# google-research/frame-interpolation

Measured on NVIDIA H100. Metric: interpolated_frames_per_sec_1080p, higher is better.
Workload: dtype f16x2-split (activations/weights as fp16 hi+lo planes; fp32 accumulate)

## Files before the change

### frame_interpolation_b200/csrc/film_conv.h

```cpp
#pragma once
#include <cuda.h>
#include <stdint.h>

#include "film_common.cuh"

namespace film {

constexpr int kMaxSrc = 4;
constexpr int kMaxTaps = 9;
constexpr int kChunk = 64;
constexpr int kTileM = 128;

struct ConvSrc {
  const sp_t* hi;
  const sp_t* lo;
  int C;
  int c_off;
  int nchunk;
  int bswap;
};

struct alignas(64) ConvProblem {
  CUtensorMap tm_a_hi[kMaxSrc];
  CUtensorMap tm_a_lo[kMaxSrc];
  CUtensorMap tm_w_hi;
  CUtensorMap tm_w_lo;
  CUtensorMap tm_w_hi_half;
  CUtensorMap tm_w_lo_half;
  ConvSrc src[kMaxSrc];
  int nsrc;
  int B, H, W;
  int tile_h, tile_w;
  int tiles_y, tiles_x;
  int ntaps;
  int tap_dy[kMaxTaps], tap_dx[kMaxTaps];
  int kchunk;
  int ktot;
// ... 2 lines not shown
  const float* bias;
  int cout;
  int act;
  sp_t* out_hi;
  sp_t* out_lo;
  int out_C, out_c_off;
  int out_H, out_W;
  int out_sy, out_sx, out_oy, out_ox;
  int epi_mode;
  const float* head_w3;
  const float* head_b3;
  int crop_y, crop_x, crop_h, crop_w;
  int64_t crop_pitch;
  const float* head_w4;
  const float* head_b4;
  const float* head_vup;
  float* head_res;
  float* head_v;
  int v2_resident;
  int v2_na, v2_nw;
  int v2_grid;
  int v2_part_lo, v2_part_hi;
  sp_t* pool_hi;
  sp_t* pool_lo;
  int pool_C;
  int group;
  int pair;
  int halo;
  int bn;
  int passes;
  int straight;
  int out_lo_skip;
  int pxn;
};

cudaError_t launch_conv_tc(const ConvProblem* d_prob, const ConvProblem& h_prob, cudaStream_t st);
cudaError_t launch_conv_simt(const ConvProblem* d_prob, const ConvProblem& h_prob, cudaStream_t st);
cudaError_t conv_tc_configure();
bool conv3x3_tc_plan(ConvProblem& h_prob, int num_sms);
void conv3x3_tc_pick_tile(int H, int W, int B, int cout, int kc, int passes, int ktot, int epi_mode, int num_sms,
                          int& tile_h, int& tile_w);
cudaError_t launch_conv3x3_tc(const ConvProblem* d_prob, const ConvProblem& h_prob, cudaStream_t st);
cudaError_t conv3x3_tc_configure();
}
```

### frame_interpolation_b200/csrc/film_conv3x3_tc.cu

```cuda
#include <cuda.h>
#include <cuda_runtime.h>
#include <stdint.h>

#include <type_traits>

#include "film_conv.h"
#include "film_tc_ptx.cuh"

namespace film {
namespace {
using namespace tc;

constexpr int kConsumers = 256;
constexpr int kThreads = kConsumers + 128;
__host__ __device__ constexpr int a_plane_bytes(int kc, int th, int tw) { return (th + 2) * tw * kc * 2; }
__host__ __device__ constexpr int a_stage_bytes(int kc, int th, int tw) { return 2 * a_plane_bytes(kc, th, tw); }
constexpr int kHaloW = 10;
__host__ __device__ constexpr int halo_box_bytes(int kc, int th) { return (th + 2) * kHaloW * kc * 2; }
__host__ __device__ constexpr int halo_plane_bytes(int kc, int th) { return (halo_box_bytes(kc, th) + 1023) & ~1023; }
__host__ __device__ constexpr int a_stage_bytes_h(int kc, int th, int tw, int halo, int planes = 2) {
  return planes * (halo ? halo_plane_bytes(kc, th) : a_plane_bytes(kc, th, tw));
}
constexpr int kMaxRing = 8;
constexpr int kSmemLimit = 227 * 1024;
// ... 537 lines not shown
              f0 = leaky(f0);
              f1 = leaky(f1);
            }
            if (valid[h]) {
              sp_t* oh = out_hi + opix[h] * out_C + out_c_off + n0;
              if (lo_skip) {
                *reinterpret_cast<uint32_t*>(oh + c) = pack2_hi(f0, f1);
              } else {
                sp_t* ol = out_lo + opix[h] * out_C + out_c_off + n0;
                uint32_t hi, lo;
                split_pack2(f0, f1, hi, lo);
                *reinterpret_cast<uint32_t*>(oh + c) = hi;
                *reinterpret_cast<uint32_t*>(ol + c) = lo;
              }
            }
            if (do_pool) {
              a[h][0] = f0 + __shfl_xor_sync(0xffffffffu, f0, 4);
              a[h][1] = f1 + __shfl_xor_sync(0xffffffffu, f1, 4);
            }
          }
          if (do_pool && pool_ok) {
            uint32_t hi, lo;
            split_pack2((a[0][0] + a[1][0]) * 0.25f, (a[0][1] + a[1][1]) * 0.25f, hi, lo);
            *reinterpret_cast<uint32_t*>(pool_hi + ppix * pool_C + n0 + c) = hi;
            *reinterpret_cast<uint32_t*>(pool_lo + ppix * pool_C + n0 + c) = lo;
          }
        }
      }
    }
  }
  leave();
}

int smem_bytes_for(const ConvProblem& h, int bn) {
  const int nkb = h.ktot / h.kchunk;
  const int planes = h.passes == 1 ? 1 : 2;
  const int w = h.v2_resident ? nkb * w_tap_bytes(bn, h.kchunk, planes) : h.v2_nw * w_tap_bytes(bn, h.kchunk, planes);
  return h.v2_na * a_stage_bytes_h(h.kchunk, h.tile_h, h.tile_w, h.halo, planes) + w + kFixedBytes +
         epi_scratch_bytes(h.epi_mode, h.pxn);
}

}

int conv_tc_block_n(int cout);

namespace {
bool ring_depths(int kc, int tile_h, int tile_w, int halo, int planes, int bn, int cout, int ktot, int epi_mode, int pxn,
                 int& resident, int& na, int& nw) {
  const int wtap = w_tap_bytes(bn, kc, planes);
  const int w_all = (ktot / kc) * wtap;
  const int kLimit = kSmemLimit - epi_scratch_bytes(epi_mode, pxn);
  const int kAStage = a_stage_bytes_h(kc, tile_h, tile_w, halo, planes);
  if (cout <= bn && w_all + 2 * kAStage + kFixedBytes <= kLimit) {
    resident = 1;
    const int n = (kLimit - kFixedBytes - w_all) / kAStage;
    const int n_max = halo ? 3 : 6;
    na = n > n_max ? n_max : n;
    nw = 1;
    return true;
  }
  resident = 0;
  na = halo ? 2 : (bn >= 128 ? 2 : 3);
  int n = (kLimit - kFixedBytes - na * kAStage) / wtap;
  if (n < 2 && na > 2) {
    na = 2;
    n = (kLimit - kFixedBytes - na * kAStage) / wtap;
// ... 75 lines not shown
    if (h.v2_na < 2 || (!h.v2_resident && h.v2_nw < 2)) return cudaErrorInvalidValue;
    if (kPxN && (h.pair || h.tile_h != 32 || h.tile_w != 8 || h.epi_mode != 0)) return cudaErrorInvalidValue;
    const bool partial = h.v2_part_hi > h.v2_part_lo;
    const int idx = (partial ? 8 : 0) | (h.halo ? 4 : 0) | (h.passes == 1 ? 2 : 0) | (h.v2_resident && h.straight ? 1 : 0);
    if (!h.pair) {
      kFn[idx]<<<h.v2_grid, kThreads, smem_bytes_for(h, BN), st>>>(d_prob);
      return cudaGetLastError();
    }
    cudaLaunchConfig_t cfg = {};
    cudaLaunchAttribute attr[1];
    attr[0].id = cudaLaunchAttributeClusterDimension;
    attr[0].val.clusterDim.x = 2;
    attr[0].val.clusterDim.y = 1;
    attr[0].val.clusterDim.z = 1;
    cfg.gridDim = dim3(h.v2_grid);
    cfg.blockDim = dim3(kThreads);
    cfg.dynamicSmemBytes = smem_bytes_for(h, BN);
    cfg.stream = st;
    cfg.attrs = attr;
    cfg.numAttrs = 1;
    return cudaLaunchKernelEx(&cfg, kFn[idx], d_prob);
  }
};

cudaError_t conv3x3_tc_configure() {
  cudaError_t e;
#define FILM_CFG(BN, KC)                        \
  e = Variants<BN, KC>::configure();            \
  if (e != cudaSuccess) return e;
  FILM_CFG(32, 64) FILM_CFG(64, 64) FILM_CFG(128, 64) FILM_CFG(256, 64) FILM_CFG(32, 32) FILM_CFG(64, 32)
#undef FILM_CFG
  e = Variants<64, 64, true>::configure();
  if (e != cudaSuccess) return e;
  return cudaSuccess;
}

cudaError_t launch_conv3x3_tc(const ConvProblem* d_prob, const ConvProblem& h, cudaStream_t st) {
  const int bn = h.bn;
  if (h.kchunk == 32) {
    if (bn == 32) return Variants<32, 32>::launch(d_prob, h, st);
    if (bn == 64) return Variants<64, 32>::launch(d_prob, h, st);
    return cudaErrorInvalidValue;
  }
  switch (bn) {
    case 256: return Variants<256, 64>::launch(d_prob, h, st);
    case 128: return Variants<128, 64>::launch(d_prob, h, st);
    case 64: return h.pxn ? Variants<64, 64, true>::launch(d_prob, h, st) : Variants<64, 64>::launch(d_prob, h, st);
    default: return Variants<32, 64>::launch(d_prob, h, st);
  }
}

}
```

### frame_interpolation_b200/csrc/film_engine.cu

```cuda
#include <cuda.h>
#include <cuda_runtime.h>

#include <algorithm>
#include <cmath>
#include <cstdio>
#include <cstdlib>
#include <cstring>
#include <functional>
#include <map>
#include <memory>
#include <string>
#include <vector>

#include "../../include/film_b200.h"
#include "film_conv.h"
#include "film_kernels.h"
#include "film_pack.h"

namespace film {
int conv_tc_block_n(int cout);

constexpr int kLevels = 7, kFusionLevels = 5, kSpecialized = 3, kSubLevels = 4, kFilters = 64;
static const int kFlowFilters[4] = {32, 64, 128, 256};
static const char* kPredictorNames[4] = {"flow_predictor_0", "flow_predictor_1", "flow_predictor_2",
// ... 22 lines not shown
static std::string stage_name(int s) {
  static const char* fe[] = {"fe_i0_k01", "fe_i0_k23", "fe_i0_k45", "fe_i0_k67", "fe_i1", "fe_i2", "fe_i3p"};
  if (s < 0 || s >= ST_COUNT) return "";
  if (s < ST_FLOW_L0) return fe[s];
  if (s < ST_FUS) return "flow_L" + std::to_string(s - ST_FLOW_L0);
  return "fus" + std::to_string((s - ST_FUS) / 3) + "_c" + std::to_string((s - ST_FUS) % 3);
}
static int fe_stage(int image_level, int conv_k) {
  if (image_level == 0) return ST_FE_I0_K01 + conv_k / 2;
  return image_level == 1 ? ST_FE_I1 : image_level == 2 ? ST_FE_I2 : ST_FE_I3P;
}
constexpr uint32_t kDefaultOnepassMask =
    (1u << ST_FE_I0_K23) | (1u << ST_FE_I0_K45) | (1u << ST_FE_I0_K67) |
    (0x1Fu << ST_FLOW_L0) | (0x3Fu << (ST_FUS + 6));

struct Options {
  int conv_impl = 0;
  int use_graph = 1;
  int keep_debug = 0;
  int time_ops = 0;
  int use_lanes = 0;
  int conv3x3_v2 = 1;
  int conv3x3_2cta = 0;
  int conv3x3_halo = 3;
  int conv3x3_pxn = 1;
  int onepass_mask = (int)kDefaultOnepassMask;
  int fe_conv0_tc = 0;
  int fuse_rgb_head = 1;
  int fuse_flow_head = 1;
  int plane_skip = 1;
  int mma_straight = 1;
  int arena_reuse = 1;
  int any_size = 0;
};

static int as_given(int v) { return v; }
static int as_bool(int v) { return v ? 1 : 0; }
static int clamp_0_2(int v) { return v < 0 ? 0 : (v > 2 ? 2 : v); }
static int stage_bits(int v) { return (int)((uint32_t)v & ((1u << ST_COUNT) - 1u)); }
struct OptionRow {
  const char* name;
  int Options::*field;
  int (*normalise)(int);
  const char* env;
  bool plan_key;
};
static const OptionRow kOptions[] = {
    {"conv_impl", &Options::conv_impl, as_given, nullptr, true},
    {"use_graph", &Options::use_graph, as_given, nullptr, false},
    {"keep_debug", &Options::keep_debug, as_given, nullptr, true},
    {"time_ops", &Options::time_ops, as_given, nullptr, false},
    {"use_lanes", &Options::use_lanes, as_given, nullptr, true},
    {"conv3x3_v2", &Options::conv3x3_v2, as_given, nullptr, true},
    {"conv3x3_2cta", &Options::conv3x3_2cta, as_given, "FILM_2CTA", true},
    {"conv3x3_halo", &Options::conv3x3_halo, as_given, "FILM_HALO", true},
    {"conv3x3_pxn", &Options::conv3x3_pxn, clamp_0_2, nullptr, true},
    {"onepass_mask", &Options::onepass_mask, stage_bits, "FILM_ONEPASS", true},
    {"fe_conv0_tc", &Options::fe_conv0_tc, as_bool, "FILM_FE0_TC", true},
    {"fuse_rgb_head", &Options::fuse_rgb_head, as_bool, "FILM_RGB_FUSE", true},
    {"fuse_flow_head", &Options::fuse_flow_head, clamp_0_2, "FILM_FLOW_HEAD_FUSE", true},
    {"plane_skip", &Options::plane_skip, as_bool, "FILM_PLANE_SKIP", true},
    {"mma_straight", &Options::mma_straight, as_bool, "FILM_STRAIGHT", true},
    {"arena_reuse", &Options::arena_reuse, as_bool, "FILM_ARENA_REUSE", true},
    {"any_size", &Options::any_size, as_bool, nullptr, false},
};
static const OptionRow& option_row(const char* name) {
  for (const OptionRow& r : kOptions)
    if (!strcmp(r.name, name)) return r;
  throw Error{FILM_ERR_ARG, std::string("unknown option ") + name};
}

#define FILM_CUDA(expr)                                                                       \
  do {                                                                                        \
    cudaError_t e__ = (expr);                                                                 \
    if (e__ != cudaSuccess)                                                                   \
      throw Error{FILM_ERR_CUDA, std::string(#expr) + ": " + cudaGetErrorString(e__)};        \
  } while (0)

struct HostTensor {
  std::vector<int> dims;
  std::vector<float> data;
};
typedef std::map<std::string, HostTensor> WeightMap;

static WeightMap read_weight_file(const char* path) {
  FILE* f = fopen(path, "rb");
  if (!f) throw Error{FILM_ERR_WEIGHTS, std::string("cannot open weight file ") + path};
  WeightMap m;
  auto fail = [&](const char* why) {
    fclose(f);
    throw Error{FILM_ERR_WEIGHTS, std::string(path) + ": " + why};
  };
  char magic[8];
  if (fread(magic, 1, 8, f) != 8 || memcmp(magic, "FILMW1\0\0", 8) != 0) fail("bad magic");
  uint32_t n;
  if (fread(&n, 4, 1, f) != 1) fail("truncated");
  for (uint32_t i = 0; i < n; ++i) {
// ... 50 lines not shown
}
static float sp_to_f32(uint16_t h) {
#ifdef FILM_SPLIT_FP16
  __half v;
  memcpy(&v, &h, 2);
  return __half2float(v);
#else
  return bf16_to_f32(h);
#endif
}

struct PackedConv {
  sp_t* w_hi = nullptr;
  sp_t* w_lo = nullptr;
  float* bias = nullptr;
  int cout = 0, ktot = 0, cin_ref = 0;
  int kchunk = kChunk;
  std::vector<int> src_chunks;
  std::vector<int> src_ksteps;
  sp_t* pxn_hi = nullptr;
  sp_t* pxn_lo = nullptr;
  int pxn_ktot = 0;
  int ntaps = 0;
  int tap_dy[kMaxTaps], tap_dx[kMaxTaps];
};

struct TapSpec {
  int dy, dx;
  std::vector<std::pair<int, int>> terms;
};

static PackedConv pack_conv(const HostTensor& kernel, const HostTensor& bias,
                            const std::vector<std::vector<int>>& src_maps,
                            const std::vector<TapSpec>& taps, std::vector<void*>& allocs, int chunk = kChunk) {
  const int kw = kernel.dims[1], cin = kernel.dims[2], cout = kernel.dims[3];
  PackedConv pc;
  pc.cout = cout;
  pc.cin_ref = cin;
  pc.kchunk = chunk;
  pc.ntaps = (int)taps.size();
  for (size_t t = 0; t < taps.size(); ++t) {
    pc.tap_dy[t] = taps[t].dy;
    pc.tap_dx[t] = taps[t].dx;
  }
  int ktot = 0;
  for (auto& sm : src_maps) {
    if (sm.size() % chunk) throw Error{FILM_ERR_WEIGHTS, "source channel map not a multiple of the K chunk"};
    pc.src_chunks.push_back((int)sm.size() / chunk);
    int ks = 1;
    for (size_t i = 0; i < sm.size(); ++i)
      if (sm[i] >= 0) ks = std::max(ks, (int)(i % chunk) / 16 + 1);
    pc.src_ksteps.push_back(ks);
    ktot += (int)sm.size() * (int)taps.size();
  }
  pc.ktot = ktot;
  std::vector<uint16_t> hi((size_t)cout * ktot), lo((size_t)cout * ktot);
  int kbase = 0;
  for (auto& sm : src_maps) {
    const int nchunk = (int)sm.size() / chunk;
    for (int ch = 0; ch < nchunk; ++ch) {
      for (size_t t = 0; t < taps.size(); ++t, kbase += chunk) {
        for (int c = 0; c < chunk; ++c) {
          const int ref = sm[ch * chunk + c];
          for (int n = 0; n < cout; ++n) {
            float w = 0.f;
            if (ref >= 0) {
              if (ref >= cin) throw Error{FILM_ERR_WEIGHTS, "channel map out of range"};
              for (auto& term : taps[t].terms)
                w += kernel.data[(((size_t)term.first * kw + term.second) * cin + ref) * cout + n];
            }
            const uint16_t h = f32_to_sp(w);
            const uint16_t l = f32_to_sp(w - sp_to_f32(h));
            hi[(size_t)n * ktot + kbase + c] = h;
            lo[(size_t)n * ktot + kbase + c] = l;
          }
        }
      }
    }
  }
  auto upload = [&](const std::vector<uint16_t>& v) {
    sp_t* d;
    FILM_CUDA(cudaMalloc(&d, v.size() * 2));
    allocs.push_back(d);
    FILM_CUDA(cudaMemcpy(d, v.data(), v.size() * 2, cudaMemcpyHostToDevice));
    return d;
  };
  pc.w_hi = upload(hi);
  pc.w_lo = upload(lo);
  pc.pxn_hi = pc.w_hi;
  pc.pxn_lo = pc.w_lo;
  pc.pxn_ktot = ktot;
  std::vector<int> packed;
  for (int ks : pc.src_ksteps) packed.push_back(taps.size() == 9 && chunk == kChunk && ks == 1);
  if (std::count(packed.begin(), packed.end(), 1)) {
    pc.pxn_hi = upload(pack_dx_blocks(hi, cout, ktot, chunk, pc.src_chunks, packed, pc.pxn_ktot));
    pc.pxn_lo = upload(pack_dx_blocks(lo, cout, ktot, chunk, pc.src_chunks, packed, pc.pxn_ktot));
  }
  FILM_CUDA(cudaMalloc(&pc.bias, cout * 4));
  allocs.push_back(pc.bias);
  FILM_CUDA(cudaMemcpy(pc.bias, bias.data.data(), cout * 4, cudaMemcpyHostToDevice));
  return pc;
}

static std::vector<TapSpec> taps_3x3() {
  std::vector<TapSpec> t;
  for (int kx = 0; kx < 3; ++kx)
    for (int ky = 0; ky < 3; ++ky) t.push_back({ky - 1, kx - 1, {{ky, kx}}});
  return t;
}
static std::vector<TapSpec> taps_up2x2(int py, int px) {
  std::vector<TapSpec> t;
  for (int dy = 0; dy <= py; ++dy)
    for (int dx = 0; dx <= px; ++dx) {
      TapSpec s{dy, dx, {}};
      for (int fy = 0; fy < 2; ++fy)
        for (int fx = 0; fx < 2; ++fx)
          if ((py + fy) / 2 == dy && (px + fx) / 2 == dx) s.terms.push_back({fy, fx});
      t.push_back(s);
    }
  return t;
}
static std::vector<int> iota_map(int start, int n, int padded) {
  std::vector<int> m(padded, -1);
  for (int i = 0; i < n; ++i) m[i] = start + i;
  return m;
}
static std::vector<int> side_map(int C) {
  std::vector<int> m(kChunk, -1);
  for (int c = 0; c < 3; ++c) m[c] = c;
  for (int c = 0; c < 3; ++c) m[3 + c] = 3 + C + c;
  m[6] = 6 + 2 * C;
  m[7] = 7 + 2 * C;
  m[8] = 8 + 2 * C;
  m[9] = 9 + 2 * C;
  return m;
}

struct Model {
  std::vector<void*> allocs;
  float *conv0_w = nullptr, *conv0_b = nullptr;
  PackedConv fe[8];
  PackedConv fe0_3x3;
  PackedConv flow[4][3];
  PackedConv flow_c3[4];
  float *flow_w3[4], *flow_b3[4], *flow_w4[4], *flow_b4[4];
  PackedConv fus_up[4][4];
  PackedConv fus_up_2x2[4];
  PackedConv fus_c1[4], fus_c2[4];
  float *rgb_w = nullptr, *rgb_b = nullptr;

  float* upload(const HostTensor& t) {
    float* d;
    FILM_CUDA(cudaMalloc(&d, t.data.size() * 4));
    allocs.push_back(d);
    FILM_CUDA(cudaMemcpy(d, t.data.data(), t.data.size() * 4, cudaMemcpyHostToDevice));
    return d;
  }

  void load(const WeightMap& w) {
    const std::string fe_pre = "feat_net/sub_extractor/cfeat_conv_";
    conv0_w = upload(get_tensor(w, fe_pre + "0/kernel", {3, 3, 3, 64}));
    conv0_b = upload(get_tensor(w, fe_pre + "0/bias", {64}));
    {
      HostTensor k0 = get_tensor(w, fe_pre + "0/kernel", {3, 3, 3, 64});
      k0.dims = {1, 1, 27, 64};
      fe[0] = pack_conv(k0, get_tensor(w, fe_pre + "0/bias", {64}), {iota_map(0, 27, 32)},
                        {TapSpec{0, 0, {{0, 0}}}}, allocs, 32);
      fe0_3x3 = pack_conv(get_tensor(w, fe_pre + "0/kernel", {3, 3, 3, 64}), get_tensor(w, fe_pre + "0/bias", {64}),
                          {iota_map(0, 3, 32)}, taps_3x3(), allocs, 32);
    }
    int cin = 64;
    for (int k = 1; k < 8; ++k) {
      const int c = kFilters << (k / 2);
      fe[k] = pack_conv(get_tensor(w, fe_pre + std::to_string(k) + "/kernel", {3, 3, cin, c}),
                        get_tensor(w, fe_pre + std::to_string(k) + "/bias", {c}),
                        {iota_map(0, cin, cin)}, taps_3x3(), allocs);
      cin = c;
    }
    for (int p = 0; p < 4; ++p) {
      const std::string pre = std::string("predict_flow/") + kPredictorNames[p] + "/conv_";
      const int nf = kFlowFilters[p], C = feat_channels(p);
      flow[p][0] = pack_conv(get_tensor(w, pre + "0/kernel", {3, 3, 2 * C, nf}),
                             get_tensor(w, pre + "0/bias", {nf}),
                             {iota_map(0, C, C), iota_map(C, C, C)}, taps_3x3(), allocs);
      const int kc = nf < kChunk ? 32 : kChunk;
      for (int k = 1; k < 3; ++k)
        flow[p][k] = pack_conv(get_tensor(w, pre + std::to_string(k) + "/kernel", {3, 3, nf, nf}),
                               get_tensor(w, pre + std::to_string(k) + "/bias", {nf}),
                               {iota_map(0, nf, round_up(nf, kc))}, taps_3x3(), allocs, kc);
      flow_c3[p] = pack_conv(get_tensor(w, pre + "3/kernel", {1, 1, nf, nf / 2}),
                             get_tensor(w, pre + "3/bias", {nf / 2}), {iota_map(0, nf, round_up(nf, kc))},
                             {TapSpec{0, 0, {{0, 0}}}}, allocs, kc);
      flow_w3[p] = upload(get_tensor(w, pre + "3/kernel", {1, 1, nf, nf / 2}));
      flow_b3[p] = upload(get_tensor(w, pre + "3/bias", {nf / 2}));
      flow_w4[p] = upload(get_tensor(w, pre + "4/kernel", {1, 1, nf / 2, 2}));
      flow_b4[p] = upload(get_tensor(w, pre + "4/bias", {2}));
    }
    for (int i = 0; i < kFusionLevels - 1; ++i) {
      const std::string pre = "fusion/level_" + std::to_string(i) + "/conv_";
      const int nf = fusion_filters(i), C = feat_channels(i);
      const bool from_pyr = (i == kFusionLevels - 2);
      const int Cc = feat_channels(i + 1);
      const int coarse_c = from_pyr ? 2 * (3 + Cc) + 4 : fusion_filters(i + 1);
      const HostTensor& k0 = get_tensor(w, pre + "0/kernel", {2, 2, coarse_c, nf});
      const HostTensor& b0 = get_tensor(w, pre + "0/bias", {nf});
      std::vector<std::vector<int>> up_src;
      if (from_pyr)
        up_src = {iota_map(3, Cc, Cc), iota_map(6 + Cc, Cc, Cc), side_map(Cc)};
      else
        up_src = {iota_map(0, coarse_c, coarse_c)};
      for (int py = 0; py < 2; ++py)
        for (int px = 0; px < 2; ++px)
          fus_up[i][py * 2 + px] = pack_conv(k0, b0, up_src, taps_up2x2(py, px), allocs);
      fus_up_2x2[i] = pack_conv(k0, b0, up_src, {{0, 0, {{0, 0}}}, {0, 1, {{0, 1}}}, {1, 0, {{1, 0}}}, {1, 1, {{1, 1}}}},
                                allocs);
      const int a_c = 2 * (3 + C) + 4;
      fus_c1[i] = pack_conv(get_tensor(w, pre + "1/kernel", {3, 3, a_c + nf, nf}),
                            get_tensor(w, pre + "1/bias", {nf}),
                            {iota_map(3, C, C), iota_map(6 + C, C, C), side_map(C),
                             iota_map(a_c, nf, round_up(nf, kChunk))},
                            taps_3x3(), allocs);
      fus_c2[i] = pack_conv(get_tensor(w, pre + "2/kernel", {3, 3, nf, nf}),
                            get_tensor(w, pre + "2/bias", {nf}),
                            {iota_map(0, nf, round_up(nf, kChunk))}, taps_3x3(), allocs);
    }
    rgb_w = upload(get_tensor(w, "fusion/output_conv/kernel", {1, 1, 64, 3}));
    rgb_b = upload(get_tensor(w, "fusion/output_conv/bias", {3}));
  }
  ~Model() {
    for (void* p : allocs) cudaFree(p);
  }
};

typedef CUresult (*EncodeTiledFn)(CUtensorMap*, CUtensorMapDataType, cuuint32_t, void*, const cuuint64_t*,
                                  const cuuint64_t*, const cuuint32_t*, const cuuint32_t*,
                                  CUtensorMapInterleave, CUtensorMapSwizzle, CUtensorMapL2promotion,
                                  CUtensorMapFloatOOBfill);
static EncodeTiledFn get_encode_fn() {
  static EncodeTiledFn fn = nullptr;
  if (!fn) {
    void* p = nullptr;
    cudaDriverEntryPointQueryResult qres;
    FILM_CUDA(cudaGetDriverEntryPoint("cuTensorMapEncodeTiled", &p, cudaEnableDefault, &qres));
    if (qres != cudaDriverEntryPointSuccess || !p)
      throw Error{FILM_ERR_CUDA, "cuTensorMapEncodeTiled entry point not available"};
    fn = (EncodeTiledFn)p;
// ... 290 lines not shown
                                              tag + ")"};
      cp.v2_part_lo = ab;
      cp.v2_part_hi = ab + pc.src_chunks[s] * nst;
    }
  }
  const size_t idx = P.h_probs.size();
  P.h_probs.push_back(cp);
  double k_issued = 0;
  for (size_t si = 0; si < pc.src_chunks.size(); ++si)
    k_issued += (double)pc.src_chunks[si] * pc.ntaps * (v2 ? pc.src_ksteps[si] * 16 : pc.kchunk);
  P.mma_flops += (double)cp.passes * 2.0 * (double)cp.B * cp.tiles_y * cp.tiles_x * (cp.tile_h * cp.tile_w) * k_issued *
                 (double)(((pc.cout + bn - 1) / bn) * bn);
  double alg_bytes = 0;
  {
    const double px = (double)cp.B * cp.H * cp.W, planes_in = cp.passes == 1 ? 1.0 : 2.0;
    for (size_t si = 0; si < pc.src_chunks.size(); ++si) alg_bytes += px * pc.src_chunks[si] * pc.kchunk * 2.0 * planes_in;
    if (out) alg_bytes += px * pc.cout * 2.0 * (cp.out_lo_skip ? 1.0 : 2.0);
    if (pool_out) alg_bytes += px / 4.0 * pc.cout * 4.0;
    if (epi_mode == 2) alg_bytes += px * 12.0;
    if (!out && epi_mode != 2) alg_bytes += px * 24.0;
    alg_bytes += (double)pc.cout * ktot * 2.0 * planes_in;
  }
  P.last_conv_bytes = alg_bytes;
  if (no_op) return idx;
  Plan* pp = &P;
  const int impl = o.conv_impl;
  P.add_op(0, tag, [pp, idx, impl, v2](cudaStream_t st) {
    if (impl == 1) return launch_conv_simt(pp->d_probs + idx, pp->h_probs[idx], st);
    return v2 ? launch_conv3x3_tc(pp->d_probs + idx, pp->h_probs[idx], st)
              : launch_conv_tc(pp->d_probs + idx, pp->h_probs[idx], st);
  }, 2.0 * ref_macs_per_px * (double)cp.B * cp.H * cp.W, alg_bytes);
  P.ops.back().form = impl == 1 ? "simt" : !v2 ? "tc" : cp.pxn ? "3x3_pxn" : "3x3";
  return idx;
}

static void padded_size(int h, int w, int align, int& H, int& W, int& off_y, int& off_x) {
  int ph = 0, pw = 0;
  if (align > 0) {
    ph = (h % align) ? align - h % align : 0;
    pw = (w % align) ? align - w % align : 0;
  }
  H = h + ph;
  W = w + pw;
  off_y = ph / 2;
  off_x = pw / 2;
}

static std::unique_ptr<Plan> build_plan(const Model& M, int h, int w, int align, const Options& opt, int num_sms) {
  std::unique_ptr<Plan> pl(new Plan);
  Plan& P = *pl;
  P.opt = opt;
  P.reuse = !opt.keep_debug && !opt.use_lanes && opt.arena_reuse;
  const bool fuse_rgb = opt.conv_impl == 0 && opt.conv3x3_v2 && opt.fuse_rgb_head && !opt.keep_debug;
  P.h = h;
  P.w = w;
  P.num_sms = num_sms;
  padded_size(h, w, align, P.H, P.W, P.off_y, P.off_x);
  int Hs[kLevels], Ws[kLevels];
  for (int l = 0; l < kLevels; ++l) {
    Hs[l] = P.H >> l;
    Ws[l] = P.W >> l;
  }
  if (Hs[kLevels - 2] < 2 || Ws[kLevels - 2] < 2) throw Error{FILM_ERR_ARG, "frame too small"};

  P.xin = P.alloc<float>((int64_t)2 * h * w * 3, true);
  P.xout = P.alloc<float>((int64_t)h * w * 3, true);
// ... 238 lines not shown
    const int nf = fusion_filters(i), hh = Hs[i], ww = Ws[i];
    const int cpad = round_up(nf, kChunk);
    SplitBuf* up = P.split(1, hh, ww, cpad);
    std::vector<SrcRef> up_src;
    if (i == kFusionLevels - 2)
      up_src = {{batch_view(wf[i + 1], 0), 0}, {batch_view(wf[i + 1], 1), 0}, {side[i + 1], 0}};
    else
      up_src = {{net, 0}};
    if (hh != 2 * Hs[i + 1] || ww != 2 * Ws[i + 1]) {
      const bool hi_only = P.hi_only(ST_FUS + 3 * i);
      std::vector<std::pair<const SplitBuf*, SplitBuf*>> jobs;
      if (i == kFusionLevels - 2) {
        jobs.push_back({wf[i + 1], P.split(2, hh, ww, wf[i + 1]->C)});
        jobs.push_back({side[i + 1], P.split(1, hh, ww, side[i + 1]->C)});
        up_src = {{batch_view(jobs[0].second, 0), 0}, {batch_view(jobs[0].second, 1), 0}, {jobs[1].second, 0}};
      } else {
        jobs.push_back({net, P.split(1, hh, ww, net->C)});
        up_src = {{jobs[0].second, 0}};
      }
      double rbytes = 0;
      for (auto& j : jobs) rbytes += (double)j.second->pixels() * j.second->C * (hi_only ? 4.0 : 8.0);
      P.add_op(2, "fusion_resize@L" + std::to_string(i), [jobs, hi_only](cudaStream_t st) {
        for (auto& j : jobs) {
          const SplitBuf *s = j.first, *d = j.second;
          const cudaError_t e = launch_resize_nearest(s->hi, s->lo, s->C, 0, s->B, s->H, s->W, d->hi, d->lo, d->C, 0, d->H,
                                                      d->W, d->C, hi_only, st);
          if (e != cudaSuccess) return e;
        }
        return cudaSuccess;
      }, 0, rbytes);
      add_conv(P, "fusion_up@L" + std::to_string(i), 4.0 * M.fus_up_2x2[i].cin_ref * nf, M.fus_up_2x2[i], up_src, 0, up, 0,
               ST_FUS + 3 * i, ST_FUS + 3 * i + 1);
      for (auto& j : jobs) P.release(j.second);
    } else if (opt.conv_impl == 0) {
      size_t first = 0;
      for (int py = 0; py < 2; ++py)
        for (int px = 0; px < 2; ++px) {
          const size_t ci = add_conv(P, "", 0, M.fus_up[i][py * 2 + px], up_src, 0, up, 0, ST_FUS + 3 * i, ST_FUS + 3 * i + 1, 2, 2,
                                     py, px, nullptr, true);
          if (py == 0 && px == 0) first = ci;
        }
      P.h_probs[first].group = 4;
      const double up_bytes = 4.0 * P.last_conv_bytes;
      Plan* pq = &P;
      const double fl = 2.0 * 16.0 * M.fus_up[i][0].cin_ref * nf * (double)Hs[i + 1] * Ws[i + 1];
      P.add_op(0, "fusion_up@L" + std::to_string(i), [pq, first](cudaStream_t st) {
        return launch_conv_tc(pq->d_probs + first, pq->h_probs[first], st);
      }, fl, up_bytes);
    } else {
      for (int py = 0; py < 2; ++py)
        for (int px = 0; px < 2; ++px)
          add_conv(P, "fusion_up" + std::to_string(py * 2 + px) + "@L" + std::to_string(i),
                   4.0 * M.fus_up[i][0].cin_ref * nf, M.fus_up[i][py * 2 + px], up_src, 0, up, 0, ST_FUS + 3 * i,
                   ST_FUS + 3 * i + 1, 2, 2, py, px);
    }
    SplitBuf* f1 = P.split(1, hh, ww, cpad);
    SplitBuf* f2 = (fuse_rgb && i == 0) ? nullptr : P.split(1, hh, ww, cpad);
    add_conv(P, "fusion_conv1@L" + std::to_string(i), 9.0 * M.fus_c1[i].cin_ref * nf, M.fus_c1[i],
             {{batch_view(wf[i], 0), 0}, {batch_view(wf[i], 1), 0}, {side[i], 0}, {up, 0}}, 1, f1, 0, ST_FUS + 3 * i + 1,
             ST_FUS + 3 * i + 2);
    if (fuse_rgb && i == 0) {
      const size_t ci = add_conv(P, "fusion_conv2+rgb@L0", 9.0 * nf * nf + 64.0 * 3, M.fus_c2[i], {{f1, 0}}, 1, nullptr, 0,
                                 ST_FUS + 3 * i + 2, ST_NONE, 1, 1, 0, 0, nullptr, false, 2);
      ConvProblem& hp = P.h_probs[ci];
      if (hp.cout != 64 || hp.bn != 64) throw Error{FILM_ERR_UNSUPPORTED, "RGB-head epilogue expects a 64-channel N tile"};
      hp.head_w4 = M.rgb_w;
      hp.head_b4 = M.rgb_b;
      hp.head_v = P.xout;
      hp.crop_y = P.off_y;
      hp.crop_x = P.off_x;
      hp.crop_h = P.h;
      hp.crop_w = P.w;
      hp.crop_pitch = (int64_t)P.w * 3;
    } else {
      add_conv(P, "fusion_conv2@L" + std::to_string(i), 9.0 * nf * nf, M.fus_c2[i], {{f1, 0}}, 1, f2, 0, ST_FUS + 3 * i + 2,
               i > 0 ? ST_FUS + 3 * (i - 1) : ST_NONE);
    }
    if (i == kFusionLevels - 2) P.release(wf[i + 1]);
    else P.release(net);
    P.release(wf[i]);
    P.release(up);
// ... 772 lines not shown
```

### frame_interpolation_b200/csrc/film_pack.h

```cpp
#pragma once
#include <stdint.h>

#include <vector>

namespace film {

inline std::vector<uint16_t> pack_dx_blocks(const std::vector<uint16_t>& per_tap, int cout, int ktot, int chunk,
                                            const std::vector<int>& src_chunks, const std::vector<int>& packed,
                                            int& ktot_out) {
  ktot_out = ktot;
  for (size_t s = 0; s < src_chunks.size(); ++s)
    if (packed[s]) ktot_out -= src_chunks[s] * 6 * chunk;
  std::vector<uint16_t> out((size_t)cout * ktot_out, 0);
  for (int n = 0; n < cout; ++n) {
    const uint16_t* src = per_tap.data() + (size_t)n * ktot;
    uint16_t* dst = out.data() + (size_t)n * ktot_out;
    for (size_t s = 0; s < src_chunks.size(); ++s)
      for (int ch = 0; ch < src_chunks[s]; ++ch, src += 9 * chunk) {
        if (!packed[s]) {
          for (int k = 0; k < 9 * chunk; ++k) *dst++ = src[k];
          continue;
        }
        for (int t = 0; t < 9; ++t)
          for (int c = 0; c < 16; ++c) dst[(t / 3) * chunk + (t % 3) * 16 + c] = src[t * chunk + c];
        dst += 3 * chunk;
      }
  }
  return out;
}

}
```

Before: 26.01.

## Add dedicated up2x tensor-core kernel sharing input tiles across all four phases

Adds a warp-specialized TMA+wgmma kernel for the fusion upsample conv that loads one input halo tile per channel chunk and computes all four sub-pixel output classes from it. Weights are repacked so each 256-wide N tile pulls only the taps its classes need. The epilogue writes interleaved 2x outputs with vectorized stores after a quad transpose. This replaces the grouped per-class path and is meant to cut repeated activation loads and launch/tile overhead, at the cost of more shared-memory weight traffic and a new, complex code path enabled by default.

```diff
diff --git a/frame_interpolation_b200/csrc/film_conv.h b/frame_interpolation_b200/csrc/film_conv.h
--- a/frame_interpolation_b200/csrc/film_conv.h
+++ b/frame_interpolation_b200/csrc/film_conv.h
@@ -3,6 +3,7 @@
 #include <stdint.h>
 
 #include "film_common.cuh"
+#include "film_pack.h"
 
 namespace film {
 
@@ -71,6 +72,7 @@
   int straight;
   int out_lo_skip;
   int pxn;
+  Up2xPlan up;
 };
 
 cudaError_t launch_conv_tc(const ConvProblem* d_prob, const ConvProblem& h_prob, cudaStream_t st);
@@ -81,4 +83,6 @@
                           int& tile_h, int& tile_w);
 cudaError_t launch_conv3x3_tc(const ConvProblem* d_prob, const ConvProblem& h_prob, cudaStream_t st);
 cudaError_t conv3x3_tc_configure();
+bool up2x_tc_plan(ConvProblem& h_prob, int num_sms);
+cudaError_t launch_up2x_tc(const ConvProblem* d_prob, const ConvProblem& h_prob, cudaStream_t st);
 }
diff --git a/frame_interpolation_b200/csrc/film_conv3x3_tc.cu b/frame_interpolation_b200/csrc/film_conv3x3_tc.cu
--- a/frame_interpolation_b200/csrc/film_conv3x3_tc.cu
+++ b/frame_interpolation_b200/csrc/film_conv3x3_tc.cu
@@ -593,6 +593,271 @@
   leave();
 }
 
+constexpr int kUpBoxW = 9, kUpBoxH = 17;
+constexpr int kUpAPlane = (kUpBoxW * kUpBoxH * 128 + 1023) & ~1023;
+__host__ __device__ constexpr int up2x_piece(int nf) { return nf == 64 ? 64 : nf == 128 ? 128 : 256; }
+__host__ __device__ constexpr int up2x_wplane(int nf) { return up2x_piece(nf) * 128; }
+
+template <int kNf, bool kOne>
+__global__ void __launch_bounds__(kThreads, 1) k_up2x_tc(const ConvProblem* __restrict__ prob) {
+  extern __shared__ uint8_t smem_raw[];
+  constexpr int planes = kOne ? 1 : 2;
+  constexpr int kN = up2x_piece(kNf), kUpWPlane = up2x_wplane(kNf);
+  constexpr int kAStage = planes * kUpAPlane, kWSlot = planes * kUpWPlane;
+  constexpr int kLen = up2x_seq_len(kNf);
+  constexpr uint32_t kPx = 128;
+
+  const int NA = prob->v2_na, NW = prob->v2_nw;
+  const int tiles_x = prob->tiles_x, tiles_per_img = prob->tiles_y * prob->tiles_x;
+  const int n_nt = prob->up.n_nt, nchunk = prob->src[0].nchunk, c_off = prob->src[0].c_off;
+  const int ntiles = prob->B * tiles_per_img * n_nt;
+  const FastDiv div_nt(n_nt, ntiles), div_img(tiles_per_img, ntiles), div_tx(tiles_x, ntiles);
+  auto decode = [&](int tile, int round, int& sp, int& nti) {
+    div_nt.divmod(tile, sp, nti);
+    nti += round % n_nt;
+    if (nti >= n_nt) nti -= n_nt;
+  };
+
+  const uint32_t raw = smem_u32(smem_raw);
+  const uint32_t base = (raw + 1023u) & ~1023u;
+  uint8_t* gen_base = smem_raw + (base - raw);
+  const uint32_t a_base = base;
+  const uint32_t w_base = a_base + (uint32_t)NA * kAStage;
+  const uint32_t tail_off = (uint32_t)NA * kAStage + (uint32_t)NW * kWSlot;
+  const uint32_t tail = base + tail_off;
+  float* bias_smem = reinterpret_cast<float*>(gen_base + tail_off + kBarBytes + 16);
+
+  const int warp = threadIdx.x >> 5, lane = threadIdx.x & 31;
+  if (warp == 8 && lane == 0) {
+    for (int s = 0; s < kMaxRing; ++s) {
+      mbar_init(tail + 8u * s, 1);
+      mbar_init(tail + 8u * (kMaxRing + s), 2);
+      mbar_init(tail + 8u * (2 * kMaxRing + s), 1);
+      mbar_init(tail + 8u * (3 * kMaxRing + s), 2);
+    }
+    asm volatile("fence.mbarrier_init.release.cluster;" ::: "memory");
+  }
+  if (warp < 8)
+    for (int i = threadIdx.x; i < kNf; i += kConsumers) bias_smem[i] = prob->bias[i];
+  __syncthreads();
+
+  if (warp >= 8) {
+    regs_dec<40>();
+    if (warp > 8) return;
+    const CUtensorMap* tm_a_hi = &prob->tm_a_hi[0];
+    const CUtensorMap* tm_a_lo = &prob->tm_a_lo[0];
+    const CUtensorMap* tm_w_hi = &prob->tm_w_hi;
+    const CUtensorMap* tm_w_lo = &prob->tm_w_lo;
+    RingPos ra, rw;
+    for (int tile = blockIdx.x, round = 0; tile < ntiles; tile += gridDim.x, ++round) {
+      int sp, nti, b, rem, ty, tx;
+      decode(tile, round, sp, nti);
+      div_img.divmod(sp, b, rem);
+      div_tx.divmod(rem, ty, tx);
+      const int y0 = ty * prob->tile_h, x0 = tx * prob->tile_w;
+      const int nblk = prob->up.nblk[nti];
+      int row = prob->up.row0[nti];
+      for (int ch = 0; ch < nchunk; ++ch) {
+        const int st = ra.stage;
+        mbar_wait(tail + 8u * (kMaxRing + st), ra.phase ^ 1u);
+        if (elect_one()) {
+          const uint32_t sa = a_base + st * kAStage, bar = tail + 8u * st;
+          mbar_expect_tx(bar, (uint32_t)(planes * kUpBoxW * kUpBoxH * kPx));
+          tma_load_4d(sa, tm_a_hi, bar, c_off + ch * 64, x0, y0, b);
+          if (!kOne) tma_load_4d(sa + kUpAPlane, tm_a_lo, bar, c_off + ch * 64, x0, y0, b);
+        }
+        __syncwarp();
+        ra.advance(NA);
+        for (int blk = 0; blk < nblk; ++blk) {
+          const int width = up2x_seq_width(kNf, blk % kLen);
+          for (int p = 0; p < width; p += kN, row += kN) {
+            const int ws = rw.stage;
+            mbar_wait(tail + 8u * (3 * kMaxRing + ws), rw.phase ^ 1u);
+            if (elect_one()) {
+              const uint32_t sw = w_base + ws * kWSlot, bar = tail + 8u * (2 * kMaxRing + ws);
+              mbar_expect_tx(bar, (uint32_t)kWSlot);
+              for (int r = 0; r < kN; r += 64) {
+                tma_load_2d(sw + r * kPx, tm_w_hi, bar, 0, row + r);
+                if (!kOne) tma_load_2d(sw + kUpWPlane + r * kPx, tm_w_lo, bar, 0, row + r);
+              }
+            }
+            __syncwarp();
+            rw.advance(NW);
+          }
+        }
+      }
+    }
+    return;
+  }
+
+  regs_inc<232>();
+  const int wg = warp >> 2;
+  const int q = lane & 3;
+  const int H = prob->H, W = prob->W, out_H = prob->out_H, out_W = prob->out_W, out_C = prob->out_C;
+  const int out_c_off = prob->out_c_off, act = prob->act;
+  sp_t* const out_hi = prob->out_hi;
+  sp_t* const out_lo = prob->out_lo;
+  const bool lo_skip = prob->out_lo_skip != 0;
+  const bool is_leader = (threadIdx.x & 127) == 0;
+  const uint32_t a_row0 = (uint32_t)(8 * wg * kUpBoxW) * kPx;
+  constexpr uint32_t sbo = kUpBoxW * kPx;
+  RingPos ra, rw;
+  float acc[128];
+  for (int tile = blockIdx.x, round = 0; tile < ntiles; tile += gridDim.x, ++round) {
+    int sp, nti;
+    decode(tile, round, sp, nti);
+    const int nblk = prob->up.nblk[nti];
+    int taps = 0;
+    for (int b = 0; b < 4; ++b) taps |= (prob->up.tap[nti][b] & 3) << (2 * b);
+    int rel_a = -1, rel_w = -1;
+    auto retire = [&](int next_a, int next_w) {
+      wgmma_commit();
+      wgmma_wait<1>();
+      if (is_leader) {
+        if (rel_a >= 0) mbar_arrive(tail + 8u * (kMaxRing + rel_a));
+        if (rel_w >= 0) mbar_arrive(tail + 8u * (3 * kMaxRing + rel_w));
+      }
+      rel_a = next_a;
+      rel_w = next_w;
+    };
+    for (int ch = 0; ch < nchunk; ++ch) {
+      const int st = ra.stage;
+      mbar_wait(tail + 8u * st, ra.phase);
+      const uint32_t sa = a_base + st * kAStage + a_row0;
+      for (int rep = 0; rep < nblk; rep += kLen) {
+        auto block = [&](auto i_c) {
+          constexpr int i = decltype(i_c)::value;
+          constexpr int kCol = up2x_seq_col(kNf, i), kW = up2x_seq_width(kNf, i);
+          const int blk = rep + i;
+          const int t = (taps >> (2 * blk)) & 3;
+          const uint32_t off = (uint32_t)((t >> 1) * kUpBoxW + (t & 1)) * kPx;
+          const uint64_t a_hi = make_desc_sbo<64>(sa + off, sbo);
+          const uint64_t a_lo = make_desc_sbo<64>(sa + kUpAPlane + off, sbo);
+          const uint32_t first = (ch == 0 && blk == 0) ? 0u : 1u;
+#pragma unroll
+          for (int p = 0; p < kW / kN; ++p) {
+            const int ws = rw.stage;
+            mbar_wait(tail + 8u * (2 * kMaxRing + ws), rw.phase);
+            const uint32_t sw = w_base + ws * kWSlot;
+            const uint64_t w_hi = make_desc_kc<64>(sw), w_lo = make_desc_kc<64>(sw + kUpWPlane);
+            float* const d = acc + (kCol + p * kN) / 2;
+            wgmma_fence();
+#pragma unroll
+            for (int k = 0; k < 4; ++k) {
+              const uint64_t adv = (uint64_t)(k * 32 >> 4);
+              if constexpr (kOne) {
+                wgmma<kN>(d, a_hi + adv, w_hi + adv, k == 0 ? first : 1u);
+              } else {
+                wgmma<kN>(d, a_lo + adv, w_hi + adv, k == 0 ? first : 1u);
+                wgmma<kN>(d, a_hi + adv, w_lo + adv, 1u);
+                wgmma<kN>(d, a_hi + adv, w_hi + adv, 1u);
+              }
+            }
+            retire(blk == nblk - 1 && p == kW / kN - 1 ? st : -1, ws);
+            rw.advance(NW);
+          }
+        };
+        block(std::integral_constant<int, 0>{});
+        if constexpr (kLen > 1) block(std::integral_constant<int, 1>{});
+        if constexpr (kLen > 2) {
+          block(std::integral_constant<int, 2>{});
+          block(std::integral_constant<int, 3>{});
+        }
+      }
+      ra.advance(NA);
+    }
+    wgmma_wait<0>();
+    if (is_leader) {
+      if (rel_a >= 0) mbar_arrive(tail + 8u * (kMaxRing + rel_a));
+      if (rel_w >= 0) mbar_arrive(tail + 8u * (3 * kMaxRing + rel_w));
+    }
+    acc_fence<128>(acc);
+
+    int b, rem, ty, tx;
+    div_img.divmod(sp, b, rem);
+    div_tx.divmod(rem, ty, tx);
+    const int r0 = (warp & 3) * 16 + (lane >> 2);
+    const int cy = ty * prob->tile_h + 8 * wg + (r0 >> 3), cx = tx * prob->tile_w + (r0 & 7);
+#pragma unroll
+    auto quad_transpose = [&](const uint32_t (&v)[4]) {
+      uint4 r = make_uint4(0u, 0u, 0u, 0u);
+#pragma unroll
+      for (int k = 0; k < 4; ++k) {
+        const int e = (q - k) & 3, src = (q + k) & 3;
+        const uint32_t x = e == 0 ? v[0] : e == 1 ? v[1] : e == 2 ? v[2] : v[3];
+        const uint32_t got = __shfl_sync(0xffffffffu, x, (lane & ~3) | src);
+        if (src == 0) r.x = got;
+        if (src == 1) r.y = got;
+        if (src == 2) r.z = got;
+        if (src == 3) r.w = got;
+      }
+      return r;
+    };
+    if constexpr (kNf == 256) {
+      const int c0 = 0;
+      const int cl = prob->up.cls[nti], py = cl >> 1, px = cl & 1;
+#pragma unroll
+      for (int j = 0; j < 32; ++j) {
+        const int c = c0 + 8 * j + 2 * q;
+#pragma unroll
+        for (int h = 0; h < 2; ++h) {
+          const int y = cy + h, x = cx;
+          float f0 = acc[4 * j + 2 * h] + bias_smem[c], f1 = acc[4 * j + 2 * h + 1] + bias_smem[c + 1];
+          if (act) {
+            f0 = leaky(f0);
+            f1 = leaky(f1);
+          }
+          if (y < H && x < W) {
+            const int64_t o = (((int64_t)b * out_H + 2 * y + py) * out_W + 2 * x + px) * out_C + out_c_off + c;
+            if (lo_skip) {
+              *reinterpret_cast<uint32_t*>(out_hi + o) = pack2_hi(f0, f1);
+            } else {
+              uint32_t hi, lo;
+              split_pack2(f0, f1, hi, lo);
+              *reinterpret_cast<uint32_t*>(out_hi + o) = hi;
+              *reinterpret_cast<uint32_t*>(out_lo + o) = lo;
+            }
+          }
+        }
+      }
+      continue;
+    }
+#pragma unroll
+    for (int m = 0; m < 8; ++m) {
+      const int g = nti * kUp2xTile + 32 * m;
+      const int cl = prob->up.cls[g / kNf], c0 = g % kNf;
+      const int py = cl >> 1, px = cl & 1;
+#pragma unroll
+      for (int h = 0; h < 2; ++h) {
+        const int y = cy + h, x = cx;
+        uint32_t vh[4], vl[4];
+#pragma unroll
+        for (int jj = 0; jj < 4; ++jj) {
+          const int i = 4 * (4 * m + jj) + 2 * h, c = c0 + 8 * jj + 2 * q;
+          float f0 = acc[i] + bias_smem[c], f1 = acc[i + 1] + bias_smem[c + 1];
+          if (act) {
+            f0 = leaky(f0);
+            f1 = leaky(f1);
+          }
+          if (lo_skip) {
+            vh[jj] = pack2_hi(f0, f1);
+            vl[jj] = 0u;
+          } else {
+            split_pack2(f0, f1, vh[jj], vl[jj]);
+          }
+        }
+        const uint4 th = quad_transpose(vh);
+        const uint4 tl = lo_skip ? th : quad_transpose(vl);
+        if (y < H && x < W) {
+          const int64_t o = (((int64_t)b * out_H + 2 * y + py) * out_W + 2 * x + px) * out_C + out_c_off + c0 + 8 * q;
+          *reinterpret_cast<uint4*>(out_hi + o) = th;
+          if (!lo_skip) *reinterpret_cast<uint4*>(out_lo + o) = tl;
+        }
+      }
+    }
+  }
+}
+
 int smem_bytes_for(const ConvProblem& h, int bn) {
   const int nkb = h.ktot / h.kchunk;
   const int planes = h.passes == 1 ? 1 : 2;
@@ -734,7 +999,39 @@
 #undef FILM_CFG
   e = Variants<64, 64, true>::configure();
   if (e != cudaSuccess) return e;
+  for (auto fn : {k_up2x_tc<64, false>, k_up2x_tc<64, true>, k_up2x_tc<128, false>, k_up2x_tc<128, true>,
+                  k_up2x_tc<256, false>, k_up2x_tc<256, true>}) {
+    e = cudaFuncSetAttribute(fn, cudaFuncAttributeMaxDynamicSharedMemorySize, kSmemLimit);
+    if (e != cudaSuccess) return e;
+  }
   return cudaSuccess;
+}
+
+bool up2x_tc_plan(ConvProblem& h, int num_sms) {
+  const int planes = h.passes == 1 ? 1 : 2;
+  h.v2_na = planes == 1 ? 3 : 2;
+  const int n = (kSmemLimit - kFixedBytes - h.v2_na * planes * kUpAPlane) / (planes * up2x_wplane(h.up.nf));
+  h.v2_nw = n > kMaxRing ? kMaxRing : n;
+  const int items = h.B * h.tiles_y * h.tiles_x * h.up.n_nt;
+  h.v2_grid = items <= num_sms ? items : num_sms - num_sms % h.up.n_nt;
+  return h.v2_nw >= 2 && h.tile_h == 16 && h.tile_w == 8 && h.kchunk == 64 && h.nsrc == 1 && h.out_C % 8 == 0 &&
+         h.out_c_off % 8 == 0;
+}
+
+cudaError_t launch_up2x_tc(const ConvProblem* d_prob, const ConvProblem& h, cudaStream_t st) {
+  if (h.v2_na < 2 || h.v2_nw < 2) return cudaErrorInvalidValue;
+  const bool one = h.passes == 1;
+  const int planes = one ? 1 : 2;
+  const int smem = h.v2_na * planes * kUpAPlane + h.v2_nw * planes * up2x_wplane(h.up.nf) + kFixedBytes;
+  void (*fn)(const ConvProblem*) = nullptr;
+  switch (h.up.nf) {
+    case 64: fn = one ? k_up2x_tc<64, true> : k_up2x_tc<64, false>; break;
+    case 128: fn = one ? k_up2x_tc<128, true> : k_up2x_tc<128, false>; break;
+    case 256: fn = one ? k_up2x_tc<256, true> : k_up2x_tc<256, false>; break;
+    default: return cudaErrorInvalidValue;
+  }
+  fn<<<h.v2_grid, kThreads, smem, st>>>(d_prob);
+  return cudaGetLastError();
 }
 
 cudaError_t launch_conv3x3_tc(const ConvProblem* d_prob, const ConvProblem& h, cudaStream_t st) {
diff --git a/frame_interpolation_b200/csrc/film_engine.cu b/frame_interpolation_b200/csrc/film_engine.cu
--- a/frame_interpolation_b200/csrc/film_engine.cu
+++ b/frame_interpolation_b200/csrc/film_engine.cu
@@ -78,6 +78,7 @@
   int mma_straight = 1;
   int arena_reuse = 1;
   int any_size = 0;
+  int conv_up_v2 = 1;
 };
 
 static int as_given(int v) { return v; }
@@ -109,6 +110,7 @@
     {"mma_straight", &Options::mma_straight, as_bool, "FILM_STRAIGHT", true},
     {"arena_reuse", &Options::arena_reuse, as_bool, "FILM_ARENA_REUSE", true},
     {"any_size", &Options::any_size, as_bool, nullptr, false},
+    {"conv_up_v2", &Options::conv_up_v2, as_bool, nullptr, true},
 };
 static const OptionRow& option_row(const char* name) {
   for (const OptionRow& r : kOptions)
@@ -225,7 +227,8 @@
 
 static PackedConv pack_conv(const HostTensor& kernel, const HostTensor& bias,
                             const std::vector<std::vector<int>>& src_maps,
-                            const std::vector<TapSpec>& taps, std::vector<void*>& allocs, int chunk = kChunk) {
+                            const std::vector<TapSpec>& taps, std::vector<void*>& allocs, int chunk = kChunk,
+                            std::vector<uint16_t>* keep_hi = nullptr, std::vector<uint16_t>* keep_lo = nullptr) {
   const int kw = kernel.dims[1], cin = kernel.dims[2], cout = kernel.dims[3];
   PackedConv pc;
   pc.cout = cout;
@@ -280,6 +283,8 @@
   };
   pc.w_hi = upload(hi);
   pc.w_lo = upload(lo);
+  if (keep_hi) *keep_hi = hi;
+  if (keep_lo) *keep_lo = lo;
   pc.pxn_hi = pc.w_hi;
   pc.pxn_lo = pc.w_lo;
   pc.pxn_ktot = ktot;
@@ -338,6 +343,11 @@
   PackedConv flow_c3[4];
   float *flow_w3[4], *flow_b3[4], *flow_w4[4], *flow_b4[4];
   PackedConv fus_up[4][4];
+  struct Up2xWeights {
+    Up2xPlan plan;
+    bool ok = false;
+    sp_t *w_hi = nullptr, *w_lo = nullptr;
+  } fus_up2x[4];
   PackedConv fus_up_2x2[4];
   PackedConv fus_c1[4], fus_c2[4];
   float *rgb_w = nullptr, *rgb_b = nullptr;
@@ -402,9 +412,23 @@
         up_src = {iota_map(3, Cc, Cc), iota_map(6 + Cc, Cc, Cc), side_map(Cc)};
       else
         up_src = {iota_map(0, coarse_c, coarse_c)};
+      std::vector<uint16_t> cls_hi[4], cls_lo[4];
       for (int py = 0; py < 2; ++py)
         for (int px = 0; px < 2; ++px)
-          fus_up[i][py * 2 + px] = pack_conv(k0, b0, up_src, taps_up2x2(py, px), allocs);
+          fus_up[i][py * 2 + px] = pack_conv(k0, b0, up_src, taps_up2x2(py, px), allocs, kChunk, &cls_hi[py * 2 + px],
+                                             &cls_lo[py * 2 + px]);
+      Up2xWeights& u = fus_up2x[i];
+      u.ok = up_src.size() == 1 && up2x_plan(nf, coarse_c / kChunk, u.plan);
+      if (u.ok) {
+        for (auto* v : {&cls_hi, &cls_lo}) {
+          const std::vector<uint16_t> packed = pack_up2x(*v, u.plan);
+          sp_t* d;
+          FILM_CUDA(cudaMalloc(&d, packed.size() * 2));
+          allocs.push_back(d);
+          FILM_CUDA(cudaMemcpy(d, packed.data(), packed.size() * 2, cudaMemcpyHostToDevice));
+          (v == &cls_hi ? u.w_hi : u.w_lo) = d;
+        }
+      }
       fus_up_2x2[i] = pack_conv(k0, b0, up_src, {{0, 0, {{0, 0}}}, {0, 1, {{0, 1}}}, {1, 0, {{1, 0}}}, {1, 1, {{1, 1}}}},
                                 allocs);
       const int a_c = 2 * (3 + C) + 4;
@@ -761,6 +785,58 @@
   }, 2.0 * ref_macs_per_px * (double)cp.B * cp.H * cp.W, alg_bytes);
   P.ops.back().form = impl == 1 ? "simt" : !v2 ? "tc" : cp.pxn ? "3x3_pxn" : "3x3";
   return idx;
+}
+
+static void add_up2x(Plan& P, const std::string& tag, double ref_flops, const Model::Up2xWeights& u, const PackedConv& pc0,
+                     const SplitBuf* src, const SplitBuf* out, int stage, int consumer) {
+  ConvProblem cp;
+  memset(&cp, 0, sizeof(cp));
+  cp.passes = P.onepass(stage) ? 1 : 3;
+  cp.out_lo_skip = P.hi_only(consumer) ? 1 : 0;
+  cp.nsrc = 1;
+  cp.B = src->B;
+  cp.H = src->H;
+  cp.W = src->W;
+  cp.kchunk = kChunk;
+  cp.tile_h = 16;
+  cp.tile_w = 8;
+  cp.tiles_y = (cp.H + cp.tile_h - 1) / cp.tile_h;
+  cp.tiles_x = (cp.W + cp.tile_w - 1) / cp.tile_w;
+  if (u.plan.nchunk * kChunk > src->C) throw Error{FILM_ERR_ARG, "conv source channel overrun"};
+  if (out->B != cp.B || out->H != 2 * cp.H || out->W != 2 * cp.W || u.plan.nf > out->C)
+    throw Error{FILM_ERR_ARG, "conv destination mismatch"};
+  cp.src[0] = ConvSrc{src->hi, src->lo, src->C, 0, u.plan.nchunk, 0};
+  make_act_map(&cp.tm_a_hi[0], src->hi, src->B, src->H, src->W, src->C, 17, 9, kChunk);
+  make_act_map(&cp.tm_a_lo[0], src->lo, src->B, src->H, src->W, src->C, 17, 9, kChunk);
+  cp.ktot = kChunk;
+  cp.w_hi = u.w_hi;
+  cp.w_lo = u.w_lo;
+  make_w_map(&cp.tm_w_hi, u.w_hi, u.plan.rows, kChunk, 64, kChunk);
+  make_w_map(&cp.tm_w_lo, u.w_lo, u.plan.rows, kChunk, 64, kChunk);
+  cp.bias = pc0.bias;
+  cp.cout = u.plan.nf;
+  cp.bn = kUp2xTile;
+  cp.out_hi = out->hi;
+  cp.out_lo = out->lo;
+  cp.out_C = out->C;
+  cp.out_H = out->H;
+  cp.out_W = out->W;
+  cp.out_sy = cp.out_sx = 2;
+  cp.group = 1;
+  cp.up = u.plan;
+  if (!up2x_tc_plan(cp, P.num_sms))
+    throw Error{FILM_ERR_UNSUPPORTED, "up2x conv: shared-memory rings do not fit (" + tag + ")"};
+  const size_t idx = P.h_probs.size();
+  P.h_probs.push_back(cp);
+  const double kin = (double)u.plan.nchunk * kChunk, px = (double)cp.B * cp.H * cp.W, planes_in = cp.passes == 1 ? 1.0 : 2.0;
+  P.mma_flops += (double)cp.passes * 2.0 * (double)cp.B * cp.tiles_y * cp.tiles_x * 128.0 * kin * 9.0 * u.plan.nf;
+  const double bytes = px * kin * 2.0 * planes_in + 4.0 * px * u.plan.nf * 2.0 * (cp.out_lo_skip ? 1.0 : 2.0) +
+                       (double)u.plan.rows * kChunk * 2.0 * planes_in;
+  P.last_conv_bytes = bytes;
+  Plan* pp = &P;
+  P.add_op(0, tag, [pp, idx](cudaStream_t st) { return launch_up2x_tc(pp->d_probs + idx, pp->h_probs[idx], st); },
+           ref_flops, bytes);
+  P.ops.back().form = "up2x";
 }
 
 static void padded_size(int h, int w, int align, int& H, int& W, int& off_y, int& off_x) {
@@ -1065,6 +1141,9 @@
       add_conv(P, "fusion_up@L" + std::to_string(i), 4.0 * M.fus_up_2x2[i].cin_ref * nf, M.fus_up_2x2[i], up_src, 0, up, 0,
                ST_FUS + 3 * i, ST_FUS + 3 * i + 1);
       for (auto& j : jobs) P.release(j.second);
+    } else if (opt.conv_impl == 0 && opt.conv3x3_v2 && opt.conv_up_v2 && M.fus_up2x[i].ok) {
+      add_up2x(P, "fusion_up@L" + std::to_string(i), 2.0 * 16.0 * M.fus_up[i][0].cin_ref * nf * (double)Hs[i + 1] * Ws[i + 1],
+               M.fus_up2x[i], M.fus_up[i][0], up_src[0].buf, up, ST_FUS + 3 * i, ST_FUS + 3 * i + 1);
     } else if (opt.conv_impl == 0) {
       size_t first = 0;
       for (int py = 0; py < 2; ++py)
@@ -1080,6 +1159,7 @@
       P.add_op(0, "fusion_up@L" + std::to_string(i), [pq, first](cudaStream_t st) {
         return launch_conv_tc(pq->d_probs + first, pq->h_probs[first], st);
       }, fl, up_bytes);
+      P.ops.back().form = "tc";
     } else {
       for (int py = 0; py < 2; ++py)
         for (int px = 0; px < 2; ++px)
diff --git a/frame_interpolation_b200/csrc/film_pack.h b/frame_interpolation_b200/csrc/film_pack.h
--- a/frame_interpolation_b200/csrc/film_pack.h
+++ b/frame_interpolation_b200/csrc/film_pack.h
@@ -29,4 +29,72 @@
   return out;
 }
 
+constexpr int kUp2xTile = 256;
+constexpr int up2x_seq_len(int nf) { return nf == 64 ? 4 : nf == 128 ? 2 : 1; }
+constexpr int up2x_seq_col(int nf, int i) { return nf == 64 ? (i == 0 ? 0 : i == 1 ? 64 : 128) : nf == 128 ? 128 * i : 0; }
+constexpr int up2x_seq_width(int nf, int i) { return nf == 64 ? (i == 0 ? 256 : i == 3 ? 64 : 128) : nf == 128 ? 256 >> i : 256; }
+
+struct Up2xPlan {
+  int nf, nchunk, n_nt;
+  int cls[4];
+  int nblk[4];
+  int tap[4][4];
+  int col[4][4];
+  int width[4][4];
+  int row0[4];
+  int rows;
+};
+
+inline bool up2x_plan(int nf, int nchunk, Up2xPlan& p) {
+  if (nf != 64 && nf != 128 && nf != 256) return false;
+  p = Up2xPlan{};
+  p.nf = nf;
+  p.nchunk = nchunk;
+  p.n_nt = 4 * nf / kUp2xTile;
+  static const int order64[4] = {0, 1, 3, 2}, order[4] = {0, 1, 2, 3};
+  for (int k = 0; k < 4; ++k) p.cls[k] = nf == 64 ? order64[k] : order[k];
+  int row = 0;
+  for (int nt = 0; nt < p.n_nt; ++nt) {
+    p.row0[nt] = row;
+    for (int t = 0; t < 4; ++t) {
+      int lo = -1, hi = -1;
+      for (int c = 0; c < kUp2xTile; c += nf) {
+        const int cl = p.cls[(nt * kUp2xTile + c) / nf];
+        if ((t >> 1) <= (cl >> 1) && (t & 1) <= (cl & 1)) {
+          if (lo < 0) lo = c;
+          else if (hi != c) return false;
+          hi = c + nf;
+        }
+      }
+      if (lo < 0) continue;
+      const int b = p.nblk[nt]++, i = b % up2x_seq_len(nf);
+      if (lo != up2x_seq_col(nf, i) || hi - lo != up2x_seq_width(nf, i)) return false;
+      p.tap[nt][b] = t;
+      p.col[nt][b] = lo;
+      p.width[nt][b] = hi - lo;
+      row += nchunk * (hi - lo);
+    }
+    if (p.nblk[nt] % up2x_seq_len(nf)) return false;
+  }
+  p.rows = row;
+  return true;
 }
+
+inline std::vector<uint16_t> pack_up2x(const std::vector<uint16_t>* per_class, const Up2xPlan& p) {
+  const int kc = 64;
+  std::vector<uint16_t> out((size_t)p.rows * kc, 0);
+  uint16_t* dst = out.data();
+  for (int nt = 0; nt < p.n_nt; ++nt)
+    for (int ch = 0; ch < p.nchunk; ++ch)
+      for (int b = 0; b < p.nblk[nt]; ++b)
+        for (int r = 0; r < p.width[nt][b]; ++r, dst += kc) {
+          const int g = nt * kUp2xTile + p.col[nt][b] + r, cl = p.cls[g / p.nf], n = g % p.nf;
+          const int py = cl >> 1, px = cl & 1, dy = p.tap[nt][b] >> 1, dx = p.tap[nt][b] & 1;
+          const int ntaps = (py + 1) * (px + 1), ti = dy * (px + 1) + dx;
+          const uint16_t* src = per_class[cl].data() + (size_t)n * p.nchunk * ntaps * kc + ((size_t)ch * ntaps + ti) * kc;
+          for (int c = 0; c < kc; ++c) dst[c] = src[c];
+        }
+  return out;
+}
+
+}
```

After: 26.39, median of 6. 1.5% higher.
